# ivargr/kmer_mapper

Measured on AMD Instinct MI355X. Metric: M k-mers mapped/sec (whole node), k=31 150bp reads, higher is better.
Workload: dtype u64

## Files before the change

### kmer_mapper_amd/csrc/kmm.hip

```cpp
#include <hip/hip_runtime.h>

#include <climits>
#include <cstdarg>
#include <cstdint>
#include <cstdio>
#include <cstdlib>
#include <chrono>
#include <cstring>
#include <memory>
#include <mutex>
#include <string>
#include <thread>
#include <type_traits>
#include <utility>
#include <vector>

#include "kmm.h"
#include "kmm_radix_plan.hpp"

namespace {

thread_local std::string g_err;

int fail(int code, const char *fmt, ...)
// ... 178 lines not shown

struct PinnedBuf {
    uint8_t *p = nullptr;
    size_t bytes = 0;
    PinnedBuf() = default;
    PinnedBuf(const PinnedBuf &) = delete;
    PinnedBuf &operator=(const PinnedBuf &) = delete;
    ~PinnedBuf() { reset(); }
    void reset() { g_shelf.give(std::exchange(p, nullptr), std::exchange(bytes, 0)); }
};
constexpr size_t RING_SLOT = (size_t)16 << 20;
#ifndef KMM_RING_SLOTS
#define KMM_RING_SLOTS 8
#endif
constexpr int RING_SLOTS = KMM_RING_SLOTS;


struct TimedEvent {
    Event start, stop;
    int kernel_id = 0;
};

struct BgzfStaged {
    std::vector<unsigned long long> m_off, o_rel;
    uint64_t p = 0;
    int chain_err = 0;
    uint32_t bad_isize = 0, bad_ms = 0;
    bool hit_cap = false;
    bool staged = false;
    double ms_scan_inside = 0;
};

struct IndexStreams {
    Stream stream;
    Stream copy_stream;
};

struct RxDir16 {
    DevPtr<uint16_t> rx_pstart16;
    DevPtr<uint32_t> rx_slice_e0;
    DevPtr<uint16_t> rx_slice_fmax;
};
struct RxSlotFilter {
    DevPtr<uint32_t> rx_slots;
};
struct RxArrays : RxDir16, RxSlotFilter {
    uint64_t rx_S = 0;
    DevPtr<uint32_t> rx_pstart;
    DevPtr<uint64_t> rx_pkeys;
    DevPtr<uint64_t> rx_pkeys_raw;
    DevPtr<uint16_t> rx_pfreq;
    DevPtr<uint32_t> rx_pnodes, rx_porig, rx_ecnt, rx_ecnt_acc;
    DevPtr<uint32_t> rx_norder, rx_nnode;
    DevPtr<uint32_t> rx_occ;
};

struct kmm_index : IndexStreams, RxArrays {
    int device = 0;
    Event copied;
    DevPtr<uint4> buckets;
    DevPtr<uint4> entries;
    DevPtr<uint32_t> occ;
    bool use_occ = true;
    int occ_shift = 0;
    uint32_t bloom_words = 0;
    bool wide = false;
    bool direct_deferred = false;
    size_t direct_bytes = 0;
    size_t occ_bytes_plan = 0;
    int rx_why_not = 0;
    uint32_t *counts = nullptr;
    DevPtr<uint32_t> own_counts_buf;
    DevPtr<uint8_t> lut_default;
    DevPtr<uint8_t> lut_codes;
    DevPtr<unsigned long long> first_bad;
    DevPtr<unsigned long long> stats;
    DevPtr<unsigned long long> queue;
    bool dynamic_schedule = true;
    int dyn_chunk = 16;
    uint64_t modulo = 0, magic = 0;
    int64_t n_entries = 0, max_node_id = 0;
    Stage stage[2];
    int cur = 0;
    int n_cu = 256;
    int path = 0;
    int grid_per_cu = 64;
    bool rx_ok = false;
    RxGeometry rx_geo;
    bool rx_no_mid = false;
    bool rx_flush_sorted = true;
    uint32_t rx_max_slice = 0;
    bool rx_fits_small = false, rx_fits_mid = false;
    int rx_grid_per_cu = 2;
    int64_t rx_min_units = 0;
    int64_t rx_sub_cap = RX_SUB_CAP_MAX;
    int64_t rx_sub_cap_eff = 0;
    int rx_sub_cap_eff_age = 0;
    int64_t rx_sub_cap_last = 0;
    const uint32_t *dbg_T1 = nullptr, *dbg_item_base = nullptr;
    const uint16_t *dbg_start1 = nullptr;
    uint32_t dbg_F1 = 0, dbg_NB = 0;
    int host_pack_threads = 0;
    std::unique_ptr<kmm_hostpack::Workers> pack_pool;
    PinnedBuf pack_pinned;
    PinnedBuf ring[RING_SLOTS];
    PinnedBuf pack_bits_pinned;
    int64_t host_packed_calls = 0, host_packed_record_calls = 0;
    int64_t host_pack_slice_kb = 0;
    DevBuf bgzf_comp[2], bgzf_raw[2], bgzf_meta[2], bgzf_tabs, bgzf_err, bgzf_carry, bgzf_crc, bgzf_status;
    Event bgzf_done[2];
    Event bgzf_slot_ev[RING_SLOTS];
    bool bgzf_used[2] = {false, false};
    int bgzf_cur = 0;
    int64_t bgzf_carry_len = 0;
    BgzfStaged bgzf_pre;
    bool bgzf_pre_valid = false;
    const uint8_t *bgzf_pre_from = nullptr, *bgzf_hint_ptr = nullptr;
    int64_t bgzf_pre_n = 0, bgzf_hint_n = 0;
    int bgzf_pre_buf = 0;
    int64_t bgzf_prestaged_calls = 0;
    int64_t bgzf_head_skip = 0;
    int64_t bgzf_tail_stop = -1;
    int64_t bgzf_calls = 0, bgzf_members = 0;
    DevBuf gz_comp, gz_raw, gz_carry, gz_window, gz_tabs, gz_meta, gz_res, gz_win, gz_gmaps, gz_gwin, gz_err;
    std::vector<DevBuf> gz_arena;
    kmm_gunzip::StreamState gz_state;
    int64_t gz_carry_len = 0;
    double gz_ratio = 4.0;
    int64_t gzip_calls = 0, gzip_members = 0, gzip_chunks = 0, gzip_false_starts = 0, gzip_continuations = 0, gzip_inflated = 0;
    int dbg_gzip_chunk_kb = 0;
    DevBuf bam_tiles[2], bam_bad, bam_base, bam_ctl, bam_out;
    int32_t bam_n_ref = -1;
    uint32_t bam_excl = 0;
    int64_t bam_calls = 0, bam_records = 0, bam_excluded = 0, bam_header_bytes = 0, bam_false_starts = 0, bam_continuations = 0;
    DevBuf rs_comp, rs_raw, rs_meta, rs_err, rs_status;
    int64_t bam_n_ref_param = -1;
    int64_t dbg_bam_resync_kb = 0;
    int64_t dbg_bgzf_call_cap_kb = 0;
    int64_t flat_uniform_batches = 0;
    DevBuf sam_tiles, sam_base, sam_ctl;
    int64_t sam_calls = 0, sam_records = 0, sam_excluded = 0, sam_header_lines = 0;
    uint32_t bam_incl = 0, bam_min_mapq = 0;
    int sel_n_regions = 0, sel_keep_unplaced = 0;
// ... 44 lines not shown
};

namespace {

IndexView view_of(const kmm_index *ix)
{
    IndexView v;
    v.buckets = ix->buckets;
    v.entries = ix->entries;
    v.occ = ix->use_occ ? ix->occ : nullptr;
    v.occ_shift = ix->occ_shift;
    v.bloom_words = ix->bloom_words;
    v.wide = ix->wide ? 1 : 0;
    v.counts = ix->counts;
    v.stats = ix->stats;
    v.modulo = ix->modulo;
    v.magic = ix->magic;
    return v;
}

struct ScopedTimer {
    kmm_index *ix;
    TimedEvent ev{};
    bool active = false;
    int begin(kmm_index *ix_, int kernel_id)
    {
        ix = ix_;
        if (!ix->timing)
            return KMM_OK;
        if (!ix->ev_free.empty()) {
            ev = std::move(ix->ev_free.back());
            ix->ev_free.pop_back();
        } else {
            HIPCHK(hipEventCreate(ev.start.put()));
            HIPCHK(hipEventCreate(ev.stop.put()));
        }
        ev.kernel_id = kernel_id;
        HIPCHK(hipEventRecord(ev.start, ix->stream));
        active = true;
        return KMM_OK;
    }
    int end()
    {
        if (!active)
            return KMM_OK;
        HIPCHK(hipEventRecord(ev.stop, ix->stream));
        ix->ev_used.push_back(std::move(ev));
        active = false;
        return KMM_OK;
    }
};

int rx_flush(kmm_index *ix);
int rx_build_slots(kmm_index *ix);
bool rx_slots_active(const kmm_index *ix);
int rx_check_conservation(kmm_index *ix);
int ensure_direct(kmm_index *ix);
constexpr size_t KMM_STAT_BYTES = (size_t)KMM_STAT_SHARDS * KMM_STAT_STRIDE * 8;

int drain(kmm_index *ix)
{
    KMMCHK(rx_flush(ix));
    HIPCHK(hipStreamSynchronize(ix->copy_stream));
    HIPCHK(hipStreamSynchronize(ix->stream));
    if (ix->sticky_rc != KMM_OK)
        return fail(ix->sticky_rc, "%s", ix->sticky_msg.c_str());
    KMMCHK(rx_check_conservation(ix));
    unsigned long long bad[3] = {NO_BAD, NO_BAD, NO_BAD};
    HIPCHK(hipMemcpy(bad, ix->first_bad, sizeof bad, hipMemcpyDeviceToHost));
    if (bad[0] != NO_BAD || bad[1] != NO_BAD || bad[2] != NO_BAD) {
        unsigned long long reset[3] = {NO_BAD, NO_BAD, NO_BAD};
        HIPCHK(hipMemcpy(ix->first_bad, reset, sizeof reset, hipMemcpyHostToDevice));
        char where[160];
        snprintf(where, sizeof where, " [one of the map calls since the last synchronising call; the latest was call "
                 "#%llu on this handle; counts are invalid until kmm_reset_counts]", (unsigned long long)ix->map_calls);
        int rc;
        if (bad[2] != NO_BAD)
            rc = fail(KMM_ERR_INVALID_ARG, "read_offsets of a mapped chunk is not non-decreasing at read %llu%s",
                      bad[2], where);
        else if (bad[1] != NO_BAD)
            rc = fail(KMM_ERR_MALFORMED,
                      "record structure violated at byte offset %llu of a mapped chunk (a record line "
                      "does not start with '@' / '+' / '>'%s): multi-line FASTA/FASTQ is not supported by "
                      "the GPU reader%s", bad[1],
                      ix->min_base_quality > 0 ? ", or a quality line that ends there is not as long as its sequence line "
                                                 "(checked with min_base_quality set)" : "", where);
        else
            rc = fail(KMM_ERR_INVALID_BASE,
                      "read byte at offset %llu of a mapped chunk is not a nucleotide under the "
                      "lookup table (the reference's DNA encoder raises here)%s", bad[0], where);
        ix->sticky_rc = rc;
        ix->sticky_msg = g_err;
        return rc;
    }
    return KMM_OK;
}

int grid_for(const kmm_index *ix, int64_t work_items, int per_cu)
{
    int64_t cap = (int64_t)ix->n_cu * per_cu;
    int64_t g = work_items < cap ? work_items : cap;
    return (int)(g < 1 ? 1 : g);
}

int grid_for_tiles(const kmm_index *ix, int64_t n_tiles)
{
// ... 3880 lines not shown
        HIPCHK(hipStreamSynchronize(ix->stream));
    if (!strcmp(name, "path")) {
        if (value < 0 || value > 2)
            return fail(KMM_ERR_INVALID_ARG, "path must be 0 (auto), 1 (direct) or 2 (radix)");
        if (value == 2 && !ix->rx_ok)
            return fail(KMM_ERR_INVALID_ARG, "the radix path is not available for this index (modulo %llu: needs modulo < 2^31 "
                        "and slices whose entries fit LDS)", (unsigned long long)ix->modulo);
        ix->path = (int)value;
    } else if (!strcmp(name, "part_shift")) {
        const int rc = rx_reconfigure(ix, (int)value, -1, true);
        if (rc == RX_REFUSED)
            return fail(KMM_ERR_INVALID_ARG, "part_shift %lld: needs 0 <= shift <= 13, at most 512 x 512 fine partitions "
                        "and 2^shift small enough for the quotient of a 64-bit k-mer by the modulo to fit beside "
                        "the hash bits", (long long)value);
        KMMCHK(rc);
    } else if (!strcmp(name, "radix_packed_tiles")) {
        ix->rx_packed = value != 0;
    } else if (!strcmp(name, "radix_filter")) {
        ix->rx_filter = value != 0;
        if (ix->rx_pstart) {
            const int rc = rx_reconfigure(ix, ix->rx_geo.w, -1, false);
            if (rc != RX_REFUSED)
                KMMCHK(rc);
        }
    } else if (!strcmp(name, "radix_filter_slots")) {
        ix->rx_filter_slots = value != 0;
        if (ix->rx_pstart && ix->rx_ok)
            KMMCHK(rx_build_slots(ix));
    } else if (!strcmp(name, "radix_p3_fingerprints")) {
        ix->rx_p3_fp = value != 0;
    } else if (!strcmp(name, "debug_p2f_round_slots")) {
        if (value < 512 || value > P2F_SLOTS || (value & 1))
            return fail(KMM_ERR_INVALID_ARG, "debug_p2f_round_slots must be even and in [512, %d]", P2F_SLOTS);
        ix->dbg_p2f_cap = (uint32_t)value;
    } else if (!strcmp(name, "fine_bits")) {
        const int rc = value < 0 || value > 9 ? RX_REFUSED : rx_reconfigure(ix, ix->rx_geo.w, (int)value, true);
        if (rc == RX_REFUSED)
            return fail(KMM_ERR_INVALID_ARG, "fine_bits %lld: both fan-outs must stay within 512", (long long)value);
        KMMCHK(rc);
    } else if (!strcmp(name, "radix_min_units")) {
        ix->rx_min_units = value;
    } else if (!strcmp(name, "radix_sub_batch_kmers")) {
        if (value < 4 * RX_B || value > ((int64_t)1 << 32) - 2 * RX_B)
            return fail(KMM_ERR_INVALID_ARG, "radix_sub_batch_kmers outside [%d, 2^32 - %d]", 4 * RX_B, 2 * RX_B);
        ix->rx_sub_cap = value;
        ix->rx_sub_cap_eff = 0;
    } else if (!strcmp(name, "comm_overlap_slices")) {
        if (value < 1 || value > 64)
            return fail(KMM_ERR_INVALID_ARG, "comm_overlap_slices outside [1, 64]");
        ix->comm_slices = (int)value;
        ix->flush_cuts.clear();
    } else if (!strcmp(name, "radix_sorted_flush")) {
        ix->rx_flush_sorted = value != 0;
    } else if (!strcmp(name, "radix_grid_per_cu")) {
        if (value < 1 || value > 2)
            return fail(KMM_ERR_INVALID_ARG, "radix_grid_per_cu must be 1 or 2");
        ix->rx_grid_per_cu = (int)value;
    } else if (!strcmp(name, "count_kmers")) {
        if (value && !ix->rx_ok)
            return fail(KMM_ERR_INVALID_ARG, "count_kmers needs the radix path, which is not available for this index");
        KMMCHK(rx_flush(ix));
        HIPCHK(hipStreamSynchronize(ix->stream));
        if (value && !ix->rx_ecnt_acc) {
            const size_t S = ix->rx_S ? ix->rx_S : 1;
            HIPCHK(hipMalloc(ix->rx_ecnt_acc.put(), S * 4));
            HIPCHK(hipMemset(ix->rx_ecnt_acc, 0, S * 4));
        } else if (!value && ix->rx_ecnt_acc) {
            HIPCHK(ix->rx_ecnt_acc.reset());
        }
    } else if (!strcmp(name, "grid_per_cu")) {
        if (value < 1 || value > 1024)
            return fail(KMM_ERR_INVALID_ARG, "grid_per_cu outside [1, 1024]");
        ix->grid_per_cu = (int)value;
    } else if (!strcmp(name, "dynamic_schedule")) {
        ix->dynamic_schedule = value != 0;
    } else if (!strcmp(name, "dyn_chunk")) {
        if (value < 1 || value > 4096)
            return fail(KMM_ERR_INVALID_ARG, "dyn_chunk outside [1, 4096]");
        ix->dyn_chunk = (int)value;
    } else if (!strcmp(name, "occupancy_filter")) {
        ix->use_occ = value != 0;
    } else if (!strcmp(name, "debug_records_copy_stream")) {
        ix->dbg_rec_copy_stream = value != 0;
    } else if (!strcmp(name, "host_pack_threads")) {
        if (value < 0 || value > 256)
            return fail(KMM_ERR_INVALID_ARG, "host_pack_threads outside [0, 256]");
        ix->host_pack_threads = (int)value;
    } else if (!strcmp(name, "host_pack_slice_kb")) {
        if (value < 0 || value > 65536)
            return fail(KMM_ERR_INVALID_ARG, "host_pack_slice_kb outside [0, 65536]");
        ix->host_pack_slice_kb = value;
    } else if (!strcmp(name, "bgzf_head_skip")) {
        if (value < 0)
            return fail(KMM_ERR_INVALID_ARG, "bgzf_head_skip negative");
        ix->bgzf_head_skip = value;
    } else if (!strcmp(name, "bgzf_tail_stop")) {
        ix->bgzf_tail_stop = value < 0 ? -1 : value;
    } else if (!strcmp(name, "debug_bgzf_ring_slot_kb") || !strcmp(name, "debug_ring_slot_kb")) {
        if (value != 0 && (value < 4 || value > (1 << 20) || (value & (value - 1))))
            return fail(KMM_ERR_INVALID_ARG, "debug_ring_slot_kb: 0 or a power of two in [4, 2^20]");
        ix->dbg_bgzf_slot_kb = (int)value;
    } else if (!strcmp(name, "bam_exclude_flags")) {
        if (value < 0 || value > 0xFFFF)
            return fail(KMM_ERR_INVALID_ARG, "bam_exclude_flags outside [0, 0xFFFF]");
        ix->bam_excl = (uint32_t)value;
    } else if (!strcmp(name, "bam_include_flags")) {
// ... 173 lines not shown
    else if (!strcmp(name, "sam_records_excluded"))
        *value = ix->sam_excluded;
    else if (!strcmp(name, "sam_header_lines"))
        *value = ix->sam_header_lines;
    else if (!strcmp(name, "debug_bgzf_call_cap_kb"))
        *value = ix->dbg_bgzf_call_cap_kb;
    else if (!strcmp(name, "bam_n_ref"))
        *value = ix->bam_n_ref_param;
    else if (!strcmp(name, "debug_bam_resync_kb"))
        *value = ix->dbg_bam_resync_kb;
    else if (!strcmp(name, "flat_uniform_batches"))
        *value = ix->flat_uniform_batches;
    else if (!strcmp(name, "bgzf_members"))
        *value = ix->bgzf_members;
    else if (!strcmp(name, "bgzf_carry_bytes"))
        *value = ix->bgzf_carry_len;
    else if (!strcmp(name, "host_cpu_budget"))
        *value = kmm_hostpack::cpu_budget();
    else if (!strcmp(name, "radix_sub_batch_kmers"))
        *value = ix->rx_sub_cap;
    else if (!strcmp(name, "radix_sub_batch_kmers_effective"))
        *value = ix->rx_sub_cap_last;
    else if (!strcmp(name, "comm_overlap_slices"))
        *value = ix->comm_slices;
    else if (!strcmp(name, "comm_sliced_reduces"))
        *value = ix->comm_sliced_reduces;
    else if (!strcmp(name, "debug_rx_t1_sum") || !strcmp(name, "debug_rx_start1_sum") || !strcmp(name, "debug_rx_items")) {
        HIPCHK(hipSetDevice(ix->device));
        HIPCHK(hipStreamSynchronize(ix->copy_stream));
        HIPCHK(hipStreamSynchronize(ix->stream));
        if (!ix->dbg_T1)
            return fail(KMM_ERR_INVALID_ARG, "no radix batch has run on this handle");
        uint64_t sum = 0;
        if (name[9] == 't') {
            std::vector<uint32_t> t(ix->dbg_F1);
            HIPCHK(hipMemcpy(t.data(), ix->dbg_T1, t.size() * 4, hipMemcpyDeviceToHost));
            for (uint32_t v : t)
                sum += v;
        } else if (name[9] == 'i') {
            uint32_t v = 0;
            HIPCHK(hipMemcpy(&v, ix->dbg_item_base + ix->dbg_F1, 4, hipMemcpyDeviceToHost));
            sum = v;
        } else {
            const size_t ld = (size_t)ix->dbg_F1 + 1;
            std::vector<uint16_t> r((size_t)ix->dbg_NB * ld);
            HIPCHK(hipMemcpy(r.data(), ix->dbg_start1, r.size() * 2, hipMemcpyDeviceToHost));
            for (size_t b = 0; b < ix->dbg_NB; ++b)
                sum += r[b * ld + ld - 1];
        }
        *value = (int64_t)sum;
    }
    else if (!strcmp(name, "radix_sorted_flush"))
        *value = (ix->rx_flush_sorted && ix->rx_norder) ? 1 : 0;
    else if (!strcmp(name, "radix_available"))
        *value = ix->rx_ok ? 1 : 0;
    else if (!strcmp(name, "radix_batches"))
        *value = (int64_t)ix->n_radix_batches;
    else if (!strcmp(name, "direct_batches"))
        *value = (int64_t)ix->n_direct_batches;
    else if (!strcmp(name, "radix_unavailable_reason"))
        *value = ix->rx_ok ? 0 : ix->rx_why_not;
    else if (!strcmp(name, "direct_view_resident"))
        *value = ix->buckets ? 1 : 0;
    else if (!strcmp(name, "direct_view_bytes"))
        *value = (int64_t)ix->direct_bytes;
    else if (!strcmp(name, "radix_view_bytes"))
        *value = ix->rx_pstart ? (int64_t)rx_view_bytes(ix->modulo, ix->rx_S, ix->rx_norder != nullptr) : 0;
    else if (!strcmp(name, "radix_filter"))
        *value = (ix->rx_ok && rx_filter_active(ix)) ? 1 : 0;
    else if (!strcmp(name, "radix_p3_keys_in_lds"))
        *value = ix->rx_ok ? rx_p3_shape(rx_p3_variant(ix)).keys_in_lds : 0;
    else if (!strcmp(name, "radix_filter_buckets_per_bit"))
        *value = (ix->rx_ok && rx_filter_active(ix)) ? (1 << ix->rx_geo.occ_shift) : 0;
    else if (!strcmp(name, "radix_filter_slots"))
        *value = (ix->rx_ok && rx_slots_active(ix)) ? 1 : 0;
    else if (!strcmp(name, "radix_p3_fingerprints"))
        *value = (ix->rx_ok && rx_p3_fp_active(ix)) ? 1 : 0;
    else if (!strcmp(name, "radix_filter_bits_per_partition"))
        *value = !(ix->rx_ok && rx_filter_active(ix)) ? 0
                 : rx_slots_active(ix)                ? (int64_t)P2F_SLOT_WORDS * 32
                                                      : (int64_t)1 << (ix->rx_geo.w + ix->rx_geo.f2 - ix->rx_geo.occ_shift);
    else if (!strcmp(name, "debug_p2f_round_slots"))
        *value = ix->dbg_p2f_cap;
    else if (!strcmp(name, "radix_packed_tiles"))
        *value = ix->rx_packed ? 1 : 0;
    else if (!strcmp(name, "n_fine_per_coarse"))
        *value = ix->rx_ok ? ix->rx_geo.F2 : 0;
    else if (!strcmp(name, "count_kmers"))
        *value = ix->rx_ecnt_acc ? 1 : 0;
    else if (!strcmp(name, "n_coarse_partitions"))
        *value = ix->rx_ok ? ix->rx_geo.F1 : 0;
    else if (!strcmp(name, "radix_p2_kmers") || !strcmp(name, "radix_p3_kmers") || !strcmp(name, "radix_p2_dropped") ||
             !strcmp(name, "radix_p2_multi_round_items") || !strcmp(name, "quality_masked_bases") ||
             !strcmp(name, "records_without_qual") || !strcmp(name, "records_reversed") ||
             !strcmp(name, "debug_p3_key_reads") || !strncmp(name, "stats_slot_", 11)) {
        HIPCHK(hipSetDevice(ix->device));
        KMMCHK(drain(ix));
        std::vector<unsigned long long> st(KMM_STAT_BYTES / 8);
        HIPCHK(hipMemcpy(st.data(), ix->stats, KMM_STAT_BYTES, hipMemcpyDeviceToHost));
        const int slot = name[0] == 's' ? atoi(name + 11) : name[0] == 'q' ? KMM_STAT_QUAL_MASKED
                                                          : !strcmp(name, "records_without_qual") ? KMM_STAT_REC_NO_QUAL
                                                          : !strcmp(name, "records_reversed") ? KMM_STAT_REC_REVERSED
                                                          : name[0] == 'd' ? KMM_STAT_RX_P3_KEYS
                                                          : !strcmp(name, "radix_p2_dropped") ? KMM_STAT_RX_DROPPED
                                                          : !strcmp(name, "radix_p2_multi_round_items") ? KMM_STAT_RX_MULTI
                                                          : name[7] == '2' ? 2 : 3;
// ... 28 lines not shown
```

### kmer_mapper_amd/csrc/kmm_radix.hpp

```cpp
#pragma once
#include <type_traits>
#include "kmm_radix_plan.hpp"

constexpr int RX_NT = 512;
constexpr int RX_KPT = RX_B / RX_NT;
#ifndef RX_LPR2V
#define RX_LPR2V 16
#endif
constexpr int RX_LPR = RX_LPR2V;
constexpr int RX_NG = RX_NT / RX_LPR;
#ifndef RX_RB1
#define RX_RB1 4
#endif
#ifndef RX_RB2
#define RX_RB2 8
#endif
constexpr int RX_SUBCAP = 1024;
#ifndef RX_SUBCAP3V
#define RX_SUBCAP3V 3072
#endif
constexpr int RX_SUBCAP3 = RX_SUBCAP3V;
#ifndef RX_LPR3
#define RX_LPR3 16
#endif
// ... 1823 lines not shown
    __syncthreads();
    agg_flush_counts(iv, agg);
}

__global__ void __launch_bounds__(256) k_rx_node_hist(const uint32_t *__restrict__ pnodes, uint64_t n, uint32_t *__restrict__ hist)
{
    for (uint64_t e = (uint64_t)blockIdx.x * 256 + threadIdx.x; e < n; e += (uint64_t)gridDim.x * 256)
        atomicAdd(&hist[pnodes[e]], 1u);
}

__global__ void __launch_bounds__(256) k_rx_node_scatter(const uint32_t *__restrict__ pnodes, uint64_t n,
                                                         uint32_t *__restrict__ cursor, uint32_t *__restrict__ norder,
                                                         uint32_t *__restrict__ nnode)
{
    for (uint64_t e = (uint64_t)blockIdx.x * 256 + threadIdx.x; e < n; e += (uint64_t)gridDim.x * 256) {
        const uint32_t nd = pnodes[e];
        const uint32_t j = atomicAdd(&cursor[nd], 1u);
        norder[j] = (uint32_t)e;
        nnode[j] = nd;
    }
}

__global__ void __launch_bounds__(256) k_rx_flush_sorted(IndexView iv, const uint32_t *__restrict__ ecnt,
                                                         const uint32_t *__restrict__ norder,
                                                         const uint32_t *__restrict__ nnode, uint64_t n)
{
    constexpr int U = 4;
    const int lane = threadIdx.x & 63;
    const uint64_t n_round = (n + 255) / 256 * 256;
    for (uint64_t j0 = ((uint64_t)blockIdx.x * U) * 256 + threadIdx.x; j0 < n_round; j0 += (uint64_t)gridDim.x * U * 256) {
        uint32_t nd[U], c[U];
#pragma unroll
        for (int u = 0; u < U; ++u) {
            const uint64_t j = j0 + (uint64_t)u * 256;
            nd[u] = j < n ? nnode[j] : 0xFFFFFFFFu;
            c[u] = j < n ? ecnt[norder[j]] : 0u;
        }
#pragma unroll
        for (int u = 0; u < U; ++u) {
            uint32_t sum = c[u];
#pragma unroll
            for (int d = 1; d < 64; d <<= 1) {
                const uint32_t os = __shfl_up(sum, d), on = __shfl_up(nd[u], d);
                if (lane >= d && on == nd[u])
                    sum += os;
            }
            const uint32_t next = __shfl_down(nd[u], 1);
            if ((lane == 63 || next != nd[u]) && sum)
                atomicAdd(&iv.counts[nd[u]], sum);
        }
    }
}

__global__ void k_rx_node_cuts(const uint32_t *__restrict__ nnode, uint64_t n, const uint32_t *__restrict__ bounds, int n_bounds,
                               unsigned long long *__restrict__ cuts)
{
    for (int t = threadIdx.x; t < n_bounds; t += blockDim.x) {
        const uint32_t b = bounds[t];
        uint64_t lo = 0, hi = n;
        while (lo < hi) {
            const uint64_t mid = lo + (hi - lo) / 2;
            if (nnode[mid] < b)
                lo = mid + 1;
            else
                hi = mid;
        }
        cuts[t] = lo;
    }
}

__global__ void __launch_bounds__(256) k_rx_max_slice(const uint32_t *__restrict__ pstart, uint64_t modulo, int w,
                                                      uint32_t PF, unsigned long long *out)
{
    uint32_t m = 0, over = 0, over_mid = 0;
    for (uint64_t f = (uint64_t)blockIdx.x * 256 + threadIdx.x; f < PF; f += (uint64_t)gridDim.x * 256) {
        const uint64_t h0 = f << w, h1 = h0 + (1ull << w) < modulo ? h0 + (1ull << w) : modulo;
        const uint32_t c = pstart[h1] - pstart[h0];
        m = c > m ? c : m;
        over += c > (uint32_t)RX_ECAP ? 1u : 0u;
        over_mid += c > (uint32_t)RX_ECAP_MID ? 1u : 0u;
    }
#pragma unroll
    for (int d = 32; d > 0; d >>= 1) {
        const uint32_t o = __shfl_xor(m, d);
        m = o > m ? o : m;
        over += __shfl_xor(over, d);
        over_mid += __shfl_xor(over_mid, d);
    }
    if ((threadIdx.x & 63) == 0) {
        if (m)
            atomicMax(out, (unsigned long long)m);
        if (over)
            atomicAdd(out + 1, (unsigned long long)over);
        if (over_mid)
            atomicAdd(out + 2, (unsigned long long)over_mid);
    }
}

__global__ void k_rx_pack_keys(const uint64_t *__restrict__ raw, uint64_t n, IndexView iv, int sh,
                               uint64_t *__restrict__ packed)
{
    for (uint64_t e = (uint64_t)blockIdx.x * blockDim.x + threadIdx.x; e < n; e += (uint64_t)gridDim.x * blockDim.x) {
        uint32_t c;
        packed[e] = rx_pack(iv, sh, raw[e], &c);
    }
}
// ... 118 lines not shown
```

### kmer_mapper_amd/csrc/kmm_radix_host.hpp

```cpp
#pragma once

int rx_check_conservation(kmm_index *ix)
{
    if (!ix->rx_unchecked)
        return KMM_OK;
    ix->rx_unchecked = false;
    static thread_local std::vector<unsigned long long> st;
    st.resize(KMM_STAT_BYTES / 8);
    HIPCHK(hipMemcpy(st.data(), ix->stats, KMM_STAT_BYTES, hipMemcpyDeviceToHost));
    unsigned long long p1 = 0, p2 = 0, p3 = 0, dropped = 0;
    for (int i = 0; i < KMM_STAT_SHARDS; ++i) {
        const unsigned long long *sh = st.data() + (size_t)i * KMM_STAT_STRIDE;
        p1 += sh[KMM_STAT_RX_P1];
        p2 += sh[2];
        p3 += sh[3];
        dropped += sh[KMM_STAT_RX_DROPPED];
    }
    if (p1 == p2 && p2 == p3 + dropped)
        return KMM_OK;
    const int rc = fail(KMM_ERR_INTERNAL, "radix path self-check failed: pass 1 emitted %llu k-mers, pass 2 gathered %llu, "
                        "pass 3 probed %llu (+ %llu dropped as absent) since the counters were last reset: the node counts "
                        "are invalid until kmm_reset_counts [latest map call #%llu on this handle]",
                        p1, p2, p3, dropped, (unsigned long long)ix->map_calls);
    ix->sticky_rc = rc;
// ... 170 lines not shown
    for (int64_t s0 = 0; s0 < n_src_total; s0 += max_src) {
        const uint32_t n_src = (uint32_t)(n_src_total - s0 < max_src ? n_src_total - s0 : max_src);
        const uint32_t NB = n_src * X;
        const RxScratch sc = rx_scratch(NB, F1, F2);
        bool grew = sc.meta_bytes > ix->rx_meta.cap || sc.buf1_bytes > ix->rx_buf1.cap || sc.buf2_bytes > ix->rx_buf2.cap;
#if RX_PROBE_ANY
        grew = grew || sc.buf2_bytes > ix->rx_probe.cap;
#endif
        if (grew)
            return fail(KMM_ERR_INTERNAL, "radix path: a sub-batch of %u blocks needs more scratch than the largest one was given", NB);
        const RxView rx = rx_view_of(ix, sc, NB);
        ix->dbg_T1 = rx.T1; ix->dbg_item_base = rx.item_base; ix->dbg_start1 = rx.start1; ix->dbg_F1 = F1; ix->dbg_NB = NB;
        HIPCHK(hipMemsetAsync(rx.ctrl, 0, sc.meta_bytes - sc.ctrl, ix->stream));
        ScopedTimer tm;
        KMMCHK(tm.begin(ix, KMM_KERNEL_RX_P1));
        const int64_t tile0 = s0 * (RX_B / (MODE == MODE_RECORDS ? 1024 : 4096));
        KMMCHK(rx_launch_p1<MODE>(ix, rv, kmers_in ? kmers_in + s0 * RX_B : nullptr, n_in - s0 * RX_B, iv, rx, k, tile0, n_src,
                                  also_rc));
        HIPCHK(hipGetLastError());
        KMMCHK(tm.end());
        KMMCHK(tm.begin(ix, KMM_KERNEL_RX_SCAN));
        const bool with_p = !ix->rx_filter;
        auto chunkscan = with_p ? k_rx_chunkscan<true> : k_rx_chunkscan<false>;
        auto colscan = with_p ? k_rx_colscan<true> : k_rx_colscan<false>;
        hipLaunchKernelGGL(k_rx_colsum, dim3(sc.chunks), dim3(256), 0, ix->stream, rx);
        hipLaunchKernelGGL(chunkscan, dim3(F1), dim3(256), 0, ix->stream, rx, sc.chunks);
        hipLaunchKernelGGL(k_rx_tables, dim3(1), dim3(512), 0, ix->stream, rx);
        hipLaunchKernelGGL(colscan, dim3(sc.chunks, (F1 + 255) / 256), dim3(256), 0, ix->stream, rx);
        HIPCHK(hipGetLastError());
        KMMCHK(tm.end());
        KMMCHK(tm.begin(ix, KMM_KERNEL_RX_P2));
        rx_launch_p2(ix, iv, rx);
        HIPCHK(hipGetLastError());
        KMMCHK(tm.end());
        KMMCHK(tm.begin(ix, KMM_KERNEL_RX_SCAN));
        hipLaunchKernelGGL(k_rx_tr2, dim3((unsigned)((sc.max_items + RX_TR2 - 1) / RX_TR2)), dim3(256), 0, ix->stream, rx);
        HIPCHK(hipGetLastError());
        KMMCHK(tm.end());
        KMMCHK(tm.begin(ix, KMM_KERNEL_RX_P3));
        rx_launch_p3(ix, iv, rx, max_freq);
        HIPCHK(hipGetLastError());
        KMMCHK(tm.end());
        ix->ecnt_dirty = true;
        ix->rx_unchecked = true;
    }
    ix->n_radix_batches++;
    if (verbose && ms_since(t_0) > 20.0)
        fprintf(stderr, "libkmm: radix passes of %lld positions: %.2f ms for the batch buffers (%zu + %zu + %zu bytes), %.2f ms to issue %lld "
                "sub-batch(es)\n", (long long)units, ms_buffers, ix->rx_meta.cap, ix->rx_buf1.cap, ix->rx_buf2.cap, ms_since(t_0) - ms_buffers,
                (long long)split.n_sub);
    return KMM_OK;
}

int rx_flush(kmm_index *ix)
{
    if (!ix->ecnt_dirty)
        return KMM_OK;
    ScopedTimer tm;
    KMMCHK(tm.begin(ix, KMM_KERNEL_RX_FLUSH));
    if (ix->rx_norder && !ix->rx_ecnt_acc && ix->rx_flush_sorted) {
        hipLaunchKernelGGL(k_rx_flush_sorted, dim3(ix->n_cu * 8), dim3(256), 0, ix->stream, view_of(ix), ix->rx_ecnt,
                           ix->rx_norder, ix->rx_nnode, ix->rx_S);
        HIPCHK(hipMemsetAsync(ix->rx_ecnt, 0, (size_t)ix->rx_S * 4, ix->stream));
    } else {
        hipLaunchKernelGGL(k_rx_flush, dim3(ix->n_cu * 8), dim3(256), 0, ix->stream, view_of(ix), ix->rx_ecnt,
                           ix->rx_pnodes, ix->rx_S, ix->rx_ecnt_acc);
    }
    HIPCHK(hipGetLastError());
    KMMCHK(tm.end());
    ix->ecnt_dirty = false;
    return KMM_OK;
}

int rx_build_slots(kmm_index *ix)
{
    static_cast<RxSlotFilter &>(*ix) = RxSlotFilter();
    if (!ix->rx_filter || !ix->rx_geo.slot_filter || !ix->rx_filter_slots || !ix->rx_occ)
        return KMM_OK;
    const size_t bytes = (size_t)ix->rx_geo.F1 * P2F_SLOT_WORDS * 4;
    if (hipMalloc(ix->rx_slots.put(), bytes) != hipSuccess) {
        (void)hipGetLastError();
        static_cast<RxSlotFilter &>(*ix) = RxSlotFilter();
        return KMM_OK;
    }
    HIPCHK(hipMemsetAsync(ix->rx_slots, 0, bytes, ix->stream));
    hipLaunchKernelGGL(k_rx_build_slots, dim3(grid_for(ix, (int64_t)((ix->modulo + 255) / 256), 16)), dim3(256), 0, ix->stream,
                       ix->rx_pstart, ix->rx_pkeys, ix->modulo, ix->rx_geo.w + ix->rx_geo.f2, ix->rx_slots);
    HIPCHK(hipGetLastError());
    HIPCHK(hipStreamSynchronize(ix->stream));
    return KMM_OK;
}

int rx_repack_keys(kmm_index *ix)
{
    if (ix->rx_S)
        hipLaunchKernelGGL(k_rx_pack_keys, dim3(grid_for(ix, (int64_t)((ix->rx_S + 255) / 256), 16)), dim3(256), 0,
                           ix->stream, ix->rx_pkeys_raw, ix->rx_S, view_of(ix), ix->rx_geo.w + ix->rx_geo.f2, ix->rx_pkeys);
    HIPCHK(hipGetLastError());
    HIPCHK(hipMemsetAsync(ix->queue, 0, 3 * sizeof(unsigned long long), ix->stream));
    hipLaunchKernelGGL(k_rx_max_slice, dim3(grid_for(ix, (int64_t)((ix->rx_geo.PF + 255) / 256), 16)), dim3(256), 0, ix->stream,
                       ix->rx_pstart, ix->modulo, ix->rx_geo.w, ix->rx_geo.PF, ix->queue);
    HIPCHK(hipGetLastError());
    unsigned long long mx[3] = {0, 0, 0};
    HIPCHK(hipMemcpyAsync(mx, ix->queue, sizeof mx, hipMemcpyDeviceToHost, ix->stream));
    HIPCHK(hipStreamSynchronize(ix->stream));
    ix->rx_max_slice = (uint32_t)mx[0];
    const unsigned long long odd = ix->rx_geo.PF / 1000 > 1 ? ix->rx_geo.PF / 1000 : 1;
    ix->rx_fits_small = mx[1] <= odd;
    ix->rx_fits_mid = mx[2] <= odd;
    static_cast<RxDir16 &>(*ix) = RxDir16();
    if (ix->rx_max_slice <= 65535u && !getenv("KMM_RX_NO_P16")) {
        const size_t n16 = ((size_t)ix->rx_geo.PF << ix->rx_geo.w) + 8;
        if (hipMalloc(ix->rx_pstart16.put(), n16 * 2) == hipSuccess &&
            hipMalloc(ix->rx_slice_e0.put(), ((size_t)ix->rx_geo.PF + 2) * 4) == hipSuccess &&
            hipMalloc(ix->rx_slice_fmax.put(), ((size_t)ix->rx_geo.PF + 2) * 2) == hipSuccess) {
            hipLaunchKernelGGL(k_rx_pstart16, dim3(grid_for(ix, (int64_t)((n16 + 255) / 256), 16)), dim3(256), 0, ix->stream,
                               ix->rx_pstart, ix->modulo, ix->rx_geo.w, ix->rx_geo.PF, ix->rx_pstart16, ix->rx_slice_e0);
            HIPCHK(hipGetLastError());
            hipLaunchKernelGGL(k_rx_slice_fmax, dim3(grid_for(ix, (int64_t)((ix->rx_geo.PF + 3) / 4), 16)), dim3(256), 0, ix->stream,
                               ix->rx_slice_e0, ix->rx_pfreq, ix->rx_geo.PF, ix->rx_slice_fmax);
            HIPCHK(hipGetLastError());
            HIPCHK(hipStreamSynchronize(ix->stream));
        } else {
// ... 35 lines not shown
        if ((e = hipStreamSynchronize(ix->stream))) break;
        if (sum64 > (unsigned long long)ix->n_entries) {
            overlap = true;
            break;
        }
        if ((rc = scan_exclusive((const uint32_t *)sizes.p, ix->rx_pstart, M + 1, scratch, 0, ix->stream))) break;
        uint32_t total = 0;
        if ((e = hipMemcpyAsync(&total, ix->rx_pstart + M, 4, hipMemcpyDeviceToHost, ix->stream))) break;
        if ((e = hipStreamSynchronize(ix->stream))) break;
        ix->rx_S = total;
        {
            const size_t occ_words = (size_t)((M + 31) / 32) + ((size_t)1 << (P2F_LOGBITS + 2 - 5));
            if (hipMalloc(ix->rx_occ.put(), occ_words * 4) == hipSuccess) {
                if ((e = hipMemsetAsync(ix->rx_occ, 0, occ_words * 4, ix->stream))) break;
                hipLaunchKernelGGL(k_rx_build_occ, dim3(grid_for(ix, (int64_t)((M / 32 + 256) / 256), 16)), dim3(256), 0, ix->stream,
                                   ix->rx_pstart, M, ix->rx_occ);
            } else {
                (void)hipGetLastError();
            }
        }
        const size_t S = total ? total : 1;
        if ((e = hipMalloc(ix->rx_pkeys.put(), S * RxViewBytes::pkeys))) break;
        if ((e = hipMalloc(ix->rx_pkeys_raw.put(), S * RxViewBytes::pkeys_raw))) break;
        if ((e = hipMalloc(ix->rx_pfreq.put(), S * RxViewBytes::pfreq))) break;
        if ((e = hipMalloc(ix->rx_pnodes.put(), S * RxViewBytes::pnodes))) break;
        if ((e = hipMalloc(ix->rx_porig.put(), S * RxViewBytes::porig))) break;
        if ((e = hipMalloc(ix->rx_ecnt.put(), S * RxViewBytes::ecnt))) break;
        if ((e = hipMemsetAsync(ix->rx_ecnt, 0, S * RxViewBytes::ecnt, ix->stream))) break;
        hipLaunchKernelGGL(k_rx_pack, dim3(grid_for(ix, (int64_t)((M + 255) / 256), 16)), dim3(256), 0, ix->stream, h2i,
                           kmers, nodes, freqs, M, ix->max_node_id, ix->rx_pstart, ix->rx_pkeys_raw, ix->rx_pfreq,
                           ix->rx_pnodes, ix->rx_porig);
        if ((e = hipGetLastError())) break;
        if ((e = hipStreamSynchronize(ix->stream))) break;
        if (total) {
            const uint64_t n_nodes = (uint64_t)ix->max_node_id + 1;
            DevBuf hist, cursor;
            if (n_nodes + 1 < 0xFFFFFFFFull && (uint64_t)total / n_nodes < 8 && ensure(hist, (size_t)(n_nodes + 1) * 4) == KMM_OK &&
                ensure(cursor, (size_t)(n_nodes + 1) * 4) == KMM_OK &&
                hipMalloc(ix->rx_norder.put(), S * RxViewBytes::norder) == hipSuccess &&
                hipMalloc(ix->rx_nnode.put(), S * RxViewBytes::nnode) == hipSuccess) {
                bool ok = hipMemsetAsync(hist.p, 0, (size_t)(n_nodes + 1) * 4, ix->stream) == hipSuccess;
                hipLaunchKernelGGL(k_rx_node_hist, dim3(grid_for(ix, (int64_t)((S + 255) / 256), 16)), dim3(256), 0,
                                   ix->stream, ix->rx_pnodes, (uint64_t)total, (uint32_t *)hist.p);
                ok = ok && scan_exclusive((const uint32_t *)hist.p, (uint32_t *)cursor.p, n_nodes + 1, scratch, 0,
                                          ix->stream) == KMM_OK;
                hipLaunchKernelGGL(k_rx_node_scatter, dim3(grid_for(ix, (int64_t)((S + 255) / 256), 16)), dim3(256), 0,
                                   ix->stream, ix->rx_pnodes, (uint64_t)total, (uint32_t *)cursor.p, ix->rx_norder,
                                   ix->rx_nnode);
                ok = ok && hipGetLastError() == hipSuccess && hipStreamSynchronize(ix->stream) == hipSuccess;
                if (!ok) {
                    (void)ix->rx_norder.reset();
                    (void)ix->rx_nnode.reset();
                }
            } else {
                (void)hipGetLastError();
                (void)ix->rx_norder.reset();
                (void)ix->rx_nnode.reset();
            }
        }
    } while (0);
    (void)sizes.reset();
    scratch.clear();
    if (rc != KMM_OK || e != hipSuccess || overlap) {
        const bool nomem = rc == KMM_ERR_NOMEM || e == hipErrorOutOfMemory;
        (void)hipGetLastError();
        static_cast<RxArrays &>(*ix) = RxArrays();
        ix->rx_ok = false;
        if (overlap || nomem) {
            ix->rx_why_not = overlap ? 4 : 3;
            if (getenv("KMM_VERBOSE"))
                fprintf(stderr, "libkmm: radix view not built (%s): every batch takes the direct path\n",
                        overlap ? "the buckets of the index overlap" : "out of HBM");
            return KMM_OK;
        }
        if (rc != KMM_OK)
            return rc;
        return fail(KMM_ERR_HIP, "radix index build: %s", hipGetErrorString(e));
    }
    std::optional<int> w_force;
    if (const char *env = getenv("KMM_RX_W"))
        w_force = atoi(env);
    const int f2_force = getenv("KMM_RX_F2") ? atoi(getenv("KMM_RX_F2")) : -1;
    ix->rx_no_mid = getenv("KMM_RX_NO_MID") != nullptr;
    const std::optional<RxGeometry> geo = rx_choose_geometry(M, ix->rx_S, ix->rx_filter, w_force, f2_force);
    ix->rx_ok = geo.has_value();
    if (geo)
        ix->rx_geo = *geo;
    ix->rx_why_not = ix->rx_ok ? 0 : 2;
    if (getenv("KMM_VERBOSE"))
        fprintf(stderr, "libkmm: modulo %llu, %llu entries: radix path %s (2^%d buckets per slice, %u x %u partitions)\n",
                (unsigned long long)M, (unsigned long long)ix->rx_S, ix->rx_ok ? "available" : "NOT available: slices too "
                "dense for LDS or more than 512 x 512 of them", ix->rx_geo.w, ix->rx_geo.F1, ix->rx_geo.F2);
    if (ix->rx_ok)
        KMMCHK(rx_repack_keys(ix));
    ix->rx_min_units = rx_min_units(M, ix->rx_S);
    if (const char *env = getenv("KMM_RX_MIN_UNITS"))
        ix->rx_min_units = strtoll(env, nullptr, 10);
    return KMM_OK;
}

constexpr int RX_REFUSED = 1;
int rx_reconfigure(kmm_index *ix, int w, int f2_force, bool set_ok)
{
    const std::optional<RxGeometry> geo = rx_geometry(ix->modulo, ix->rx_S, ix->rx_filter, w, RX_MAXF, f2_force);
    if (!geo)
        return RX_REFUSED;
// ... 10 lines not shown
```

### kmer_mapper_amd/csrc/kmm_radix_plan.hpp

```cpp
#pragma once
#include <cstddef>
#include <cstdint>
#include <optional>

constexpr int RX_B = 8192;
constexpr int RX_MAXF = 512;
#ifndef RX_CHV
#define RX_CHV 256
#endif
constexpr int RX_CH = RX_CHV;
constexpr int RX_IC = 1024;
constexpr int RX_ECAP = 4096;
constexpr int RX_ECAP_BIG = 8192;
constexpr int RX_ECAP_MID = 4608;
constexpr int P2F_KMAX = 64;
constexpr int P2F_LOGBITS = 19;
constexpr int P2F_SLOT_WORDS = 3 << (P2F_LOGBITS - 6);
constexpr int P2F_SLOTS = 5888;

constexpr uint32_t rx_filter_slot(uint32_t b, uint64_t quot)
{
    const uint32_t v = ((uint32_t)quot ^ (uint32_t)(quot >> 24) ^ (uint32_t)(quot >> 48)) + (b << 23);
    const uint32_t h16 = ((v & 0xFFFFFFu) * 0x9E3779u) >> 16;
    return 3u * (b >> 1) + ((h16 * 3u) >> 16);
// ... 183 lines not shown

enum class RxP3Variant {
    W12_DIR16,
    W12,
    W13_SMALL_DIR16,
    W13_SMALL,
    W13_MID_DIR16,
    W13_MID,
    W13_BIG,
};
struct RxP3Shape {
    int keys_in_lds;
    int wg_per_cu;
    bool dir16;
    bool fingerprints = false;
};
constexpr RxP3Shape RX_P3_SHAPES[] = {
    {RX_ECAP, 2, true, true}, {RX_ECAP, 2, false},
    {RX_ECAP, 2, true}, {RX_ECAP, 2, false},
    {RX_ECAP_MID, 2, true}, {RX_ECAP_MID, 2, false},
    {RX_ECAP_BIG, 1, false},
};
constexpr const RxP3Shape &rx_p3_shape(RxP3Variant v) { return RX_P3_SHAPES[(int)v]; }
constexpr int rx_p3_fp_shapes()
{
    int n = 0;
    for (const RxP3Shape &s : RX_P3_SHAPES)
        n += s.fingerprints ? 1 : 0;
    return n;
}

inline RxP3Variant rx_choose_p3(int w, bool fits_small, bool fits_mid, bool p16, uint32_t max_slice, bool no_mid)
{
    if (w <= 12)
        return p16 ? RxP3Variant::W12_DIR16 : RxP3Variant::W12;
    const bool lds16 = p16 || max_slice <= 65535u;
    if (fits_small && lds16)
        return p16 ? RxP3Variant::W13_SMALL_DIR16 : RxP3Variant::W13_SMALL;
    if (fits_mid && lds16 && !no_mid)
        return p16 ? RxP3Variant::W13_MID_DIR16 : RxP3Variant::W13_MID;
    return RxP3Variant::W13_BIG;
}

struct RxViewBytes {
    enum : size_t { pstart = 4, pkeys = 8, pkeys_raw = 8, pfreq = 2, pnodes = 4, porig = 4, ecnt = 4, norder = 4, nnode = 4 };
};
constexpr size_t rx_view_bytes(uint64_t modulo, uint64_t S, bool node_order)
{
    return (size_t)(modulo + 1) * RxViewBytes::pstart +
           (size_t)(S ? S : 1) * (RxViewBytes::pkeys + RxViewBytes::pkeys_raw + RxViewBytes::pfreq + RxViewBytes::pnodes +
                                  RxViewBytes::porig + RxViewBytes::ecnt + (node_order ? RxViewBytes::norder + RxViewBytes::nnode : 0));
}

inline int64_t rx_min_units(uint64_t modulo, uint64_t S)
{
    const double bytes = (double)modulo * 4.0 + (double)S * 14.0;
    const double fixed = 50e-6 + bytes / 2.6e12;
    const double per_kmer_radix = 6.5e-12 * (1.0 + bytes / 40e9);
    const double per_kmer_direct = 1.0 / (bytes < 1e9 ? 60e9 : 38e9);
    const int64_t units = (int64_t)(1.25 * fixed / (per_kmer_direct - per_kmer_radix));
    return units < ((int64_t)1 << 22) ? (int64_t)1 << 22 : units;
}
```

Baseline: 178,500.

## Route radix flush through precomputed two-pass tile/range permutation tables

Replaces the sorted flush, which gathers ecnt through norder with random reads, with a two-pass routed permutation. At index build it precomputes per-tile slot tables and per-range position tables. The flush then scatters each tile into LDS, writes contiguous runs to a mid buffer, and per range permutes in LDS and does a segmented wave scan before atomically adding to node counts. It also zeroes ecnt inline, removing a separate memset. This turns random global gathers into coalesced traffic, at the cost of extra tables (about 8 bytes per entry), an extra global pass, and build-time work.

Result: no change. 179,100, median of 2 (+0.3%).

```diff
diff --git a/kmer_mapper_amd/csrc/kmm.hip b/kmer_mapper_amd/csrc/kmm.hip
--- a/kmer_mapper_amd/csrc/kmm.hip
+++ b/kmer_mapper_amd/csrc/kmm.hip
@@ -254,6 +254,8 @@
     DevPtr<uint16_t> rx_pfreq;
     DevPtr<uint32_t> rx_pnodes, rx_porig, rx_ecnt, rx_ecnt_acc;
     DevPtr<uint32_t> rx_norder, rx_nnode;
+    DevPtr<uint16_t> rx_fl_slot, rx_fl_pos, rx_fl_run, rx_fl_dst;
+    DevPtr<uint32_t> rx_fl_mid;
     DevPtr<uint32_t> rx_occ;
 };
 
@@ -291,6 +293,7 @@
     RxGeometry rx_geo;
     bool rx_no_mid = false;
     bool rx_flush_sorted = true;
+    bool rx_flush_routed = true;
     uint32_t rx_max_slice = 0;
     bool rx_fits_small = false, rx_fits_mid = false;
     int rx_grid_per_cu = 2;
@@ -441,6 +444,7 @@
 };
 
 int rx_flush(kmm_index *ix);
+bool rx_flush_routed_active(const kmm_index *ix);
 int rx_build_slots(kmm_index *ix);
 bool rx_slots_active(const kmm_index *ix);
 int rx_check_conservation(kmm_index *ix);
@@ -4427,6 +4431,8 @@
         ix->flush_cuts.clear();
     } else if (!strcmp(name, "radix_sorted_flush")) {
         ix->rx_flush_sorted = value != 0;
+    } else if (!strcmp(name, "radix_flush_routed")) {
+        ix->rx_flush_routed = value != 0;
     } else if (!strcmp(name, "radix_grid_per_cu")) {
         if (value < 1 || value > 2)
             return fail(KMM_ERR_INVALID_ARG, "radix_grid_per_cu must be 1 or 2");
@@ -4706,6 +4712,12 @@
     }
     else if (!strcmp(name, "radix_sorted_flush"))
         *value = (ix->rx_flush_sorted && ix->rx_norder) ? 1 : 0;
+    else if (!strcmp(name, "radix_flush_routed"))
+        *value = ix->rx_flush_routed ? 1 : 0;
+    else if (!strcmp(name, "radix_flush_routed_active"))
+        *value = rx_flush_routed_active(ix) ? 1 : 0;
+    else if (!strcmp(name, "radix_flush_table_bytes"))
+        *value = ix->rx_fl_slot ? (int64_t)rx_flush_plan(ix->rx_S).table_bytes : 0;
     else if (!strcmp(name, "radix_available"))
         *value = ix->rx_ok ? 1 : 0;
     else if (!strcmp(name, "radix_batches"))
diff --git a/kmer_mapper_amd/csrc/kmm_radix.hpp b/kmer_mapper_amd/csrc/kmm_radix.hpp
--- a/kmer_mapper_amd/csrc/kmm_radix.hpp
+++ b/kmer_mapper_amd/csrc/kmm_radix.hpp
@@ -1899,6 +1899,187 @@
     }
 }
 
+__global__ void __launch_bounds__(256) k_rx_flush_inverse(const uint32_t *__restrict__ norder, uint32_t n, uint32_t *__restrict__ pos)
+{
+    for (uint32_t j = blockIdx.x * 256 + threadIdx.x; j < n; j += gridDim.x * 256)
+        pos[norder[j]] = j;
+}
+
+__global__ void __launch_bounds__(1024) k_rx_flush_tab_tile(const uint32_t *__restrict__ pos, uint32_t n, uint32_t R,
+                                                            uint16_t *__restrict__ fl_slot, uint16_t *__restrict__ fl_run)
+{
+    __shared__ uint32_t lds[RXF_TILE];
+    const uint32_t base = blockIdx.x * RXF_TILE, cnt = min(n - base, RXF_TILE);
+    for (uint32_t i = threadIdx.x; i < RXF_TILE; i += 1024)
+        lds[i] = i < cnt ? (pos[base + i] / RXF_RANGE) * RXF_TILE + i : 0xFFFFFFFFu;
+    __syncthreads();
+    for (uint32_t k = 2; k <= RXF_TILE; k <<= 1)
+        for (uint32_t j = k >> 1; j > 0; j >>= 1) {
+            for (uint32_t x = threadIdx.x; x < RXF_TILE / 2; x += 1024) {
+                const uint32_t i = ((x & ~(j - 1)) << 1) | (x & (j - 1)), p = i | j;
+                const uint32_t a = lds[i], b = lds[p];
+                if ((a > b) == ((i & k) == 0)) {
+                    lds[i] = b;
+                    lds[p] = a;
+                }
+            }
+            __syncthreads();
+        }
+    for (uint32_t i = threadIdx.x; i < cnt; i += 1024)
+        fl_slot[base + (lds[i] & (RXF_TILE - 1))] = (uint16_t)i;
+    for (uint32_t r = threadIdx.x; r <= R; r += 1024) {
+        const uint32_t key = r * RXF_TILE;
+        uint32_t lo = 0, hi = cnt;
+        while (lo < hi) {
+            const uint32_t m = (lo + hi) >> 1;
+            if (lds[m] < key)
+                lo = m + 1;
+            else
+                hi = m;
+        }
+        fl_run[(size_t)blockIdx.x * (R + 1) + r] = (uint16_t)lo;
+    }
+}
+
+__global__ void __launch_bounds__(256) k_rx_flush_tab_dst(const uint16_t *__restrict__ fl_run, uint32_t T, uint32_t R,
+                                                          uint16_t *__restrict__ fl_dst)
+{
+    const uint32_t r = blockIdx.x * 256 + threadIdx.x;
+    if (r >= R)
+        return;
+    uint32_t acc = 0;
+    for (uint32_t t = 0; t < T; ++t) {
+        fl_dst[(size_t)t * R + r] = (uint16_t)acc;
+        acc += (uint32_t)fl_run[(size_t)t * (R + 1) + r + 1] - fl_run[(size_t)t * (R + 1) + r];
+    }
+}
+
+__global__ void __launch_bounds__(256) k_rx_flush_tab_pos(const uint32_t *__restrict__ pos, uint32_t n, uint32_t R,
+                                                          const uint16_t *__restrict__ fl_slot, const uint16_t *__restrict__ fl_run,
+                                                          const uint16_t *__restrict__ fl_dst, uint16_t *__restrict__ fl_pos)
+{
+    for (uint32_t e = blockIdx.x * 256 + threadIdx.x; e < n; e += gridDim.x * 256) {
+        const uint32_t p = pos[e], r = p / RXF_RANGE, t = e / RXF_TILE;
+        fl_pos[(size_t)r * RXF_RANGE + fl_dst[(size_t)t * R + r] + fl_slot[e] - fl_run[(size_t)t * (R + 1) + r]] =
+            (uint16_t)(p % RXF_RANGE);
+    }
+}
+
+__global__ void __launch_bounds__(1024) k_rx_flush_route(uint32_t *__restrict__ ecnt, uint32_t n, uint32_t T, uint32_t R,
+                                                         const uint16_t *__restrict__ fl_slot, const uint16_t *__restrict__ fl_run,
+                                                         const uint16_t *__restrict__ fl_dst, uint32_t *__restrict__ mid)
+{
+    __shared__ uint32_t lds[RXF_TILE];
+    __shared__ uint16_t s_run[RXF_MAX_RANGES], s_dst[RXF_MAX_RANGES];
+    const uint32_t per_xcd = (T + 7) / 8, t = (blockIdx.x & 7) * per_xcd + (blockIdx.x >> 3);
+    if (t >= T)
+        return;
+    const uint32_t base = t * RXF_TILE, cnt = min(n - base, RXF_TILE);
+    if (cnt == RXF_TILE) {
+        constexpr int K = RXF_TILE / 4096;
+        uint4 *e4 = reinterpret_cast<uint4 *>(ecnt + base);
+        const uint2 *s4 = reinterpret_cast<const uint2 *>(fl_slot + base);
+        uint4 v[K];
+        uint2 s[K];
+#pragma unroll
+        for (int k = 0; k < K; ++k) {
+            v[k] = e4[k * 1024 + threadIdx.x];
+            s[k] = s4[k * 1024 + threadIdx.x];
+        }
+#pragma unroll
+        for (int k = 0; k < K; ++k) {
+            e4[k * 1024 + threadIdx.x] = make_uint4(0u, 0u, 0u, 0u);
+            lds[s[k].x & 0xFFFFu] = v[k].x;
+            lds[s[k].x >> 16] = v[k].y;
+            lds[s[k].y & 0xFFFFu] = v[k].z;
+            lds[s[k].y >> 16] = v[k].w;
+        }
+    } else {
+        for (uint32_t i = threadIdx.x; i < cnt; i += 1024) {
+            lds[fl_slot[base + i]] = ecnt[base + i];
+            ecnt[base + i] = 0;
+        }
+    }
+    const uint32_t top = R > 1 ? 1u << (31 - __clz(R - 1)) : 0u, padded = top ? 2 * top : 1u;
+    for (uint32_t r = threadIdx.x; r < padded; r += 1024) {
+        s_run[r] = r < R ? fl_run[(size_t)t * (R + 1) + r] : (uint16_t)0xFFFFu;
+        s_dst[r] = r < R ? fl_dst[(size_t)t * R + r] : (uint16_t)0;
+    }
+    __syncthreads();
+    constexpr int U = 4;
+    for (uint32_t i0 = threadIdx.x; i0 < cnt; i0 += U * 1024) {
+        uint32_t lo[U];
+#pragma unroll
+        for (int u = 0; u < U; ++u)
+            lo[u] = 0;
+        for (uint32_t step = top; step; step >>= 1)
+#pragma unroll
+            for (int u = 0; u < U; ++u)
+                if (s_run[lo[u] + step] <= i0 + u * 1024)
+                    lo[u] += step;
+#pragma unroll
+        for (int u = 0; u < U; ++u) {
+            const uint32_t i = i0 + u * 1024;
+            if (i < cnt)
+                mid[(size_t)lo[u] * RXF_RANGE + s_dst[lo[u]] + (i - s_run[lo[u]])] = lds[i];
+        }
+    }
+}
+
+__global__ void __launch_bounds__(1024) k_rx_flush_apply(IndexView iv, const uint32_t *__restrict__ mid,
+                                                         const uint16_t *__restrict__ fl_pos, const uint32_t *__restrict__ nnode,
+                                                         uint32_t n)
+{
+    __shared__ uint32_t lds[RXF_RANGE];
+    const uint32_t base = blockIdx.x * RXF_RANGE, cnt = min(n - base, RXF_RANGE);
+    constexpr int J = RXF_RANGE / 1024;
+    uint32_t nd[J];
+#pragma unroll
+    for (int it = 0; it < J; ++it)
+        nd[it] = it * 1024 + threadIdx.x < cnt ? nnode[base + it * 1024 + threadIdx.x] : 0xFFFFFFFFu;
+    if (cnt == RXF_RANGE) {
+        constexpr int K = RXF_RANGE / 4096;
+        const uint4 *m4 = reinterpret_cast<const uint4 *>(mid + base);
+        const uint2 *p4 = reinterpret_cast<const uint2 *>(fl_pos + base);
+        uint4 v[K];
+        uint2 s[K];
+#pragma unroll
+        for (int k = 0; k < K; ++k) {
+            v[k] = m4[k * 1024 + threadIdx.x];
+            s[k] = p4[k * 1024 + threadIdx.x];
+        }
+#pragma unroll
+        for (int k = 0; k < K; ++k) {
+            lds[s[k].x & 0xFFFFu] = v[k].x;
+            lds[s[k].x >> 16] = v[k].y;
+            lds[s[k].y & 0xFFFFu] = v[k].z;
+            lds[s[k].y >> 16] = v[k].w;
+        }
+    } else {
+        for (uint32_t i = threadIdx.x; i < cnt; i += 1024)
+            lds[fl_pos[base + i]] = mid[base + i];
+    }
+    __syncthreads();
+    const int lane = threadIdx.x & 63;
+    const uint32_t cnt_round = (cnt + 63) & ~63u;
+#pragma unroll
+    for (int it = 0; it < J; ++it) {
+        const uint32_t j = it * 1024 + threadIdx.x;
+        if (j >= cnt_round)
+            break;
+        uint32_t sum = j < cnt ? lds[j] : 0u;
+#pragma unroll
+        for (int d = 1; d < 64; d <<= 1) {
+            const uint32_t os = __shfl_up(sum, d), on = __shfl_up(nd[it], d);
+            if (lane >= d && on == nd[it])
+                sum += os;
+        }
+        const uint32_t next = __shfl_down(nd[it], 1);
+        if ((lane == 63 || next != nd[it]) && sum)
+            atomicAdd(&iv.counts[nd[it]], sum);
+    }
+}
+
 __global__ void k_rx_node_cuts(const uint32_t *__restrict__ nnode, uint64_t n, const uint32_t *__restrict__ bounds, int n_bounds,
                                unsigned long long *__restrict__ cuts)
 {
diff --git a/kmer_mapper_amd/csrc/kmm_radix_host.hpp b/kmer_mapper_amd/csrc/kmm_radix_host.hpp
--- a/kmer_mapper_amd/csrc/kmm_radix_host.hpp
+++ b/kmer_mapper_amd/csrc/kmm_radix_host.hpp
@@ -246,13 +246,26 @@
     return KMM_OK;
 }
 
+bool rx_flush_routed_active(const kmm_index *ix)
+{
+    return ix->rx_fl_slot && ix->rx_norder && !ix->rx_ecnt_acc && ix->rx_flush_sorted && ix->rx_flush_routed &&
+           rx_flush_plan(ix->rx_S).eligible;
+}
+
 int rx_flush(kmm_index *ix)
 {
     if (!ix->ecnt_dirty)
         return KMM_OK;
     ScopedTimer tm;
     KMMCHK(tm.begin(ix, KMM_KERNEL_RX_FLUSH));
-    if (ix->rx_norder && !ix->rx_ecnt_acc && ix->rx_flush_sorted) {
+    if (rx_flush_routed_active(ix)) {
+        const RxFlushPlan fp = rx_flush_plan(ix->rx_S);
+        hipLaunchKernelGGL(k_rx_flush_route, dim3(8 * ((fp.tiles + 7) / 8)), dim3(1024), 0, ix->stream, ix->rx_ecnt, (uint32_t)ix->rx_S,
+                           fp.tiles, fp.ranges,
+                           ix->rx_fl_slot, ix->rx_fl_run, ix->rx_fl_dst, ix->rx_fl_mid);
+        hipLaunchKernelGGL(k_rx_flush_apply, dim3(fp.ranges), dim3(1024), 0, ix->stream, view_of(ix), ix->rx_fl_mid, ix->rx_fl_pos,
+                           ix->rx_nnode, (uint32_t)ix->rx_S);
+    } else if (ix->rx_norder && !ix->rx_ecnt_acc && ix->rx_flush_sorted) {
         hipLaunchKernelGGL(k_rx_flush_sorted, dim3(ix->n_cu * 8), dim3(256), 0, ix->stream, view_of(ix), ix->rx_ecnt,
                            ix->rx_norder, ix->rx_nnode, ix->rx_S);
         HIPCHK(hipMemsetAsync(ix->rx_ecnt, 0, (size_t)ix->rx_S * 4, ix->stream));
@@ -263,6 +276,38 @@
     HIPCHK(hipGetLastError());
     KMMCHK(tm.end());
     ix->ecnt_dirty = false;
+    return KMM_OK;
+}
+
+int rx_build_flush_tables(kmm_index *ix)
+{
+    auto drop = [&] {
+        (void)hipGetLastError();
+        (void)ix->rx_fl_slot.reset(); (void)ix->rx_fl_pos.reset(); (void)ix->rx_fl_run.reset(); (void)ix->rx_fl_dst.reset();
+        (void)ix->rx_fl_mid.reset();
+    };
+    drop();
+    const RxFlushPlan fp = rx_flush_plan(ix->rx_S);
+    if (!ix->rx_norder || !fp.eligible || getenv("KMM_RX_NO_FLUSH_TABLES"))
+        return KMM_OK;
+    const uint32_t S = (uint32_t)ix->rx_S;
+    DevPtr<uint32_t> pos;
+    if (hipMalloc(ix->rx_fl_slot.put(), fp.slot_bytes) != hipSuccess || hipMalloc(ix->rx_fl_pos.put(), fp.pos_bytes) != hipSuccess ||
+        hipMalloc(ix->rx_fl_run.put(), fp.run_bytes) != hipSuccess || hipMalloc(ix->rx_fl_dst.put(), fp.dst_bytes) != hipSuccess ||
+        hipMalloc(ix->rx_fl_mid.put(), fp.mid_bytes) != hipSuccess || hipMalloc(pos.put(), (size_t)S * 4) != hipSuccess) {
+        drop();
+        return KMM_OK;
+    }
+    hipLaunchKernelGGL(k_rx_flush_inverse, dim3(grid_for(ix, (int64_t)((S + 255) / 256), 16)), dim3(256), 0, ix->stream,
+                       ix->rx_norder, S, (uint32_t *)pos);
+    hipLaunchKernelGGL(k_rx_flush_tab_tile, dim3(fp.tiles), dim3(1024), 0, ix->stream, (const uint32_t *)pos, S, fp.ranges,
+                       ix->rx_fl_slot, ix->rx_fl_run);
+    hipLaunchKernelGGL(k_rx_flush_tab_dst, dim3((fp.ranges + 255) / 256), dim3(256), 0, ix->stream, ix->rx_fl_run, fp.tiles, fp.ranges,
+                       ix->rx_fl_dst);
+    hipLaunchKernelGGL(k_rx_flush_tab_pos, dim3(grid_for(ix, (int64_t)((S + 255) / 256), 16)), dim3(256), 0, ix->stream,
+                       (const uint32_t *)pos, S, fp.ranges, ix->rx_fl_slot, ix->rx_fl_run, ix->rx_fl_dst, ix->rx_fl_pos);
+    if (hipGetLastError() != hipSuccess || hipStreamSynchronize(ix->stream) != hipSuccess)
+        drop();
     return KMM_OK;
 }
 
@@ -404,6 +449,10 @@
                     (void)ix->rx_norder.reset();
                     (void)ix->rx_nnode.reset();
                 }
+                hist = DevBuf();
+                cursor = DevBuf();
+                if (ok)
+                    (void)rx_build_flush_tables(ix);
             } else {
                 (void)hipGetLastError();
                 (void)ix->rx_norder.reset();
diff --git a/kmer_mapper_amd/csrc/kmm_radix_plan.hpp b/kmer_mapper_amd/csrc/kmm_radix_plan.hpp
--- a/kmer_mapper_amd/csrc/kmm_radix_plan.hpp
+++ b/kmer_mapper_amd/csrc/kmm_radix_plan.hpp
@@ -259,6 +259,38 @@
                                   RxViewBytes::porig + RxViewBytes::ecnt + (node_order ? RxViewBytes::norder + RxViewBytes::nnode : 0));
 }
 
+constexpr uint32_t RXF_TILE = 32768, RXF_RANGE = 32768;
+constexpr uint64_t RXF_MAX_ENTRIES = (uint64_t)1 << 28;
+constexpr uint32_t RXF_MAX_RANGES = (uint32_t)(RXF_MAX_ENTRIES / RXF_RANGE);
+
+struct RxFlushPlan {
+    uint32_t tiles = 0, ranges = 0;
+    uint32_t last_tile = 0, last_range = 0;
+    size_t slot_bytes = 0, pos_bytes = 0, run_bytes = 0, dst_bytes = 0;
+    size_t table_bytes = 0;
+    size_t mid_bytes = 0;
+    bool eligible = false;
+};
+
+inline RxFlushPlan rx_flush_plan(uint64_t S)
+{
+    RxFlushPlan p;
+    if (S == 0 || S >= ((uint64_t)1 << 32))
+        return p;
+    p.tiles = (uint32_t)((S + RXF_TILE - 1) / RXF_TILE);
+    p.ranges = (uint32_t)((S + RXF_RANGE - 1) / RXF_RANGE);
+    p.last_tile = (uint32_t)(S - (uint64_t)(p.tiles - 1) * RXF_TILE);
+    p.last_range = (uint32_t)(S - (uint64_t)(p.ranges - 1) * RXF_RANGE);
+    p.slot_bytes = (size_t)S * 2;
+    p.pos_bytes = (size_t)S * 2;
+    p.run_bytes = (size_t)p.tiles * (p.ranges + 1) * 2;
+    p.dst_bytes = (size_t)p.tiles * p.ranges * 2;
+    p.table_bytes = p.slot_bytes + p.pos_bytes + p.run_bytes + p.dst_bytes;
+    p.mid_bytes = (size_t)S * 4;
+    p.eligible = S <= RXF_MAX_ENTRIES;
+    return p;
+}
+
 inline int64_t rx_min_units(uint64_t modulo, uint64_t S)
 {
     const double bytes = (double)modulo * 4.0 + (double)S * 14.0;
```
